# jstmn/cppflow

Hardware: AMD Instinct MI355X
Metric: LM-IK iterations/sec (seeds x waypoints) (higher is better)
Workload: dtype f32

## Files before the change

cppflow_amd/csrc/kernels_fused.h:

```cpp
#pragma once


__device__ __forceinline__ void load_target(const float* __restrict__ target, int w, float (&Rt)[9], float (&tt)[3]) {
    const float* t = target + (size_t)w * 7;
    tt[0] = t[0], tt[1] = t[1], tt[2] = t[2];
    quat_to_mat(t[3], t[4], t[5], t[6], Rt);
}

struct RowSummary {
    float pos_err = 0.f, rot_err = 0.f, cost = 0.f;
    int self_hit = 0, env_hit = 0, jl = 0;
};

template <int CTRL>
__device__ __forceinline__ float dpp_or_zero(float x) {
    return __builtin_bit_cast(float, __builtin_amdgcn_update_dpp(0, __builtin_bit_cast(int, x), CTRL, 0xf, 0xf, false));
}

template <bool IS_MAX>
__device__ __forceinline__ float wave_reduce_to_lane63(float v) {
    auto op = [](float a, float b) { return IS_MAX ? fmaxf(a, b) : a + b; };
    const float s1 = dpp_or_zero<0x111>(v), s2 = dpp_or_zero<0x112>(v), s3 = dpp_or_zero<0x113>(v);
    v = op(op(v, s1), op(s2, s3));
    v = op(v, dpp_or_zero<0x114>(v));
    v = op(v, dpp_or_zero<0x118>(v));
    v = op(v, dpp_or_zero<0x142>(v));
    v = op(v, dpp_or_zero<0x143>(v));
    return v;
}

__device__ __forceinline__ void lds_barrier() { asm volatile("s_waitcnt lgkmcnt(0)\n\ts_barrier" ::: "memory"); }

template <class RB>
__device__ __forceinline__ void block_seed_summary(const RB& rb, int W, size_t row, bool active, const float (&q)[RB::D],
                                                   const RowSummary& rs, float* __restrict__ out) {
    constexpr int D = RB::D;
    __shared__ float s_q[kBlock / 64][D];
    __shared__ float s_red[kBlock / 64][8];
    const int tid = threadIdx.x, lane = tid & 63, wave = tid >> 6;
    const float rad2deg = 57.29577951308232087680f;
    const int wps = W >> 6;
    if (wps > 1) {
        if (lane == 0) {
#pragma unroll
            for (int j = 0; j < D; ++j) s_q[wave][j] = q[j];
        }
        lds_barrier();
    }
    const bool seed_ends_here = ((wave + 1) & (wps - 1)) == 0;
    const bool has_next = active && !(lane == 63 && seed_ends_here);
    const int nw = wave + 1 < kBlock / 64 ? wave + 1 : wave;
    float mrev = 0.f, mpri = 0.f;
    float dq[D], wr[D];
#pragma unroll
    for (int j = 0; j < D; ++j) {
        float qn = dpp_or_zero<0x130>(q[j]);
        qn = (lane == 63) ? s_q[nw][j] : qn;
        dq[j] = wr[j] = qn - q[j];
    }
    wrap_pi_all<D>(wr);
#pragma unroll
    for (int j = 0; j < D; ++j) {
        const bool pr = rb.pris(j);
        const float a = nan_to_inf(pr ? fabsf(100.f * dq[j]) : fabsf(rad2deg * wr[j]));
        mpri = fmaxf(mpri, pr ? a : 0.f);
        mrev = fmaxf(mrev, pr ? 0.f : a);
    }
    float v[8] = {nan_to_inf(100.f * rs.pos_err), nan_to_inf(rad2deg * rs.rot_err), has_next ? mrev : 0.f, has_next ? mpri : 0.f,
                  (float)rs.self_hit, (float)rs.env_hit, (float)rs.jl, rs.cost};
#pragma unroll
    for (int k = 0; k < 8; ++k) v[k] = active ? v[k] : 0.f;
#pragma unroll
    for (int k = 0; k < 4; ++k) v[k] = wave_reduce_to_lane63<true>(v[k]);
#pragma unroll
    for (int k = 4; k < 8; ++k) v[k] = wave_reduce_to_lane63<false>(v[k]);
    float* o = out + ((uint32_t)row >> (31 - __builtin_clz((uint32_t)W))) * 8;
    if (wps == 1) {
        if (active && lane == 63) {
#pragma unroll
            for (int k = 0; k < 8; ++k) o[k] = v[k];
        }
        return;
    }
    if (lane == 63) {
#pragma unroll
        for (int k = 0; k < 8; ++k) s_red[wave][k] = v[k];
    }
    lds_barrier();
    if (active && lane == 63 && seed_ends_here) {
        for (int i = 1; i < wps; ++i) {
#pragma unroll
            for (int k = 0; k < 4; ++k) v[k] = fmaxf(v[k], s_red[wave - i][k]);
#pragma unroll
            for (int k = 4; k < 8; ++k) v[k] += s_red[wave - i][k];
        }
#pragma unroll
        for (int k = 0; k < 8; ++k) o[k] = v[k];
    }
}

#ifndef CPPF_LM_PACE
#define CPPF_LM_PACE 1
#endif
__device__ __forceinline__ void lm_pace(uint32_t t0, int k, int pace) {
    if (CPPF_LM_PACE == 0 || pace == 0) return;
    const int lag = (int)((uint32_t)__builtin_amdgcn_s_memrealtime() - t0) - k * pace, half = pace >> 1;
    if (lag > half)
        __builtin_amdgcn_s_setprio(3);
    else if (lag > 0)
        __builtin_amdgcn_s_setprio(2);
    else if (lag > -half)
        __builtin_amdgcn_s_setprio(1);
    else
        __builtin_amdgcn_s_setprio(0);
}

template <class RB>
__device__ __forceinline__ void lm_row_load(int W, const float* __restrict__ x_in, const float* __restrict__ target,
                                            size_t row, float (&q)[RB::D], float (&Rt)[9], float (&tt)[3]) {
    load_x<RB::D>(x_in, row, q);
    load_target(target, (int)((uint32_t)row % (uint32_t)W), Rt, tt);
}

#ifndef CPPF_LEAD_SINCOS
#define CPPF_LEAD_SINCOS 2
#endif
#ifndef CPPF_FIRST_LEAN
#define CPPF_FIRST_LEAN 1
#endif
template <class RB, bool LEAD, bool FIRST = false>
constexpr int lead_sincos() {
    return LEAD ? (FIRST && CPPF_LEAD_SINCOS == 2 ? 3 : CPPF_LEAD_SINCOS) : 0;
}
template <class RB, bool LEAD, bool FIRST = false>
__device__ __forceinline__ bool lm_row_iterate(const RB& rb, const LmK& prm, const cppf_lm_outputs& out, size_t row, bool last,
                                               const float (&Rt)[9], const float (&tt)[3], float* __restrict__ gate_lds,
                                               float (&q)[RB::D]) {
    constexpr int D = RB::D;
    float delta[D];
    bool conv = false;
    {
        float R[9], p[3], ax[D][3], og[D][3], J[6][D], e[6];
        fk_ee_axes<RB, lead_sincos<RB, LEAD, FIRST>()>(rb, q, R, p, ax, og);
        pose_error<LEAD>(Rt, tt, R, p, e);
        if constexpr (!LEAD) {
            if (prm.tol_pos2 > 0.f) {
                conv = dot3(e[3], e[4], e[5], e[3], e[4], e[5]) < prm.tol_pos2 && dot3(e[0], e[1], e[2], e[0], e[1], e[2]) < prm.tol_rot2;
                if (__builtin_amdgcn_ballot_w64(!conv) == 0ull) return true;
            }
        }
        jacobian_from_axes<RB>(rb, p, ax, og, J);
        float est = 0.f;
        if constexpr (D < 6) {
            lm_primal_solve<D>(J, e, prm.lm_lambda, prm.a_pos, prm.a_rot, delta);
        } else {
            float y[6];
            if constexpr (LEAD && CPPF_LEAN_BLOCK_SOLVE != 0)
                lm_dual_solve_y_blk<D>(J, e, prm.lam_r, prm.lam_p, y, est);
            else
                lm_dual_solve_y<D>(J, e, prm.lam_r, prm.lam_p, y, est);
            lm_dual_apply<D>(J, y, delta);
        }
        if constexpr (!LEAD) {
            if (last) {
                if (out.J_out) {
                    float* Jo = out.J_out + row * 6 * D;
#pragma unroll
                    for (int i = 0; i < 6; ++i)
#pragma unroll
                        for (int j = 0; j < D; ++j) Jo[i * D + j] = J[i][j] * (i < 3 ? prm.a_rot : prm.a_pos);
                }
                if (out.e_out) {
#pragma unroll
                    for (int i = 0; i < 6; ++i) out.e_out[row * 6 + i] = e[i] * (i < 3 ? prm.a_rot : prm.a_pos);
                }
            }
        }
        if constexpr (D >= 6) {
            bool flag = !conv && est > prm.gate_thr;
            if (__builtin_expect(__builtin_amdgcn_ballot_w64(flag) != 0ull, 0)) {
                if (prm.clamp && prm.gate_thr > -INFINITY) {
                    bool cut = false;
#pragma unroll
                    for (int j = 0; j < D; ++j) {
                        const float v = q[j] + delta[j];
                        cut |= (v < rb.lo(j)) | (v > rb.hi(j));
                    }
                    flag = flag && !cut;
                }
                if constexpr (LEAD) {
                    if (prm.gate_thr > -INFINITY) {
                        const float es2 = CPPF_FMA(prm.a_pos * prm.a_pos, dot3(e[3], e[4], e[5], e[3], e[4], e[5]),
                                                   prm.a_rot * prm.a_rot * dot3(e[0], e[1], e[2], e[0], e[1], e[2]));
                        flag = flag && est * est > prm.gate_rel2 * es2;
                    }
                }
                unsigned long long todo = __builtin_amdgcn_ballot_w64(flag);
                if (todo != 0ull) {
                    int rank = lm_gate_hand_over<D>(J, e, todo, gate_lds, flag);
                    lm_gate_solve<D>(prm.lam_r_d, prm.lam_p_d, todo, rank, gate_lds, flag, delta);
                    while ((todo = __builtin_amdgcn_ballot_w64(flag)) != 0ull) {
                        float R2[9], p2[3], ax2[D][3], og2[D][3], J2[6][D], e2[6];
#pragma unroll
                        for (int j = 0; j < D; ++j) asm volatile("" : "+v"(q[j]));
                        fk_ee_axes<RB, lead_sincos<RB, LEAD, FIRST>()>(rb, q, R2, p2, ax2, og2);
                        pose_error<LEAD>(Rt, tt, R2, p2, e2);
                        jacobian_from_axes<RB>(rb, p2, ax2, og2, J2);
                        rank = lm_gate_hand_over<D>(J2, e2, todo, gate_lds, flag);
                        lm_gate_solve<D>(prm.lam_r_d, prm.lam_p_d, todo, rank, gate_lds, flag, delta);
                    }
                }
            }
        }
    }
    if constexpr (!LEAD) {
        if (prm.tol_pos2 > 0.f) {
            if (!conv) {
#pragma unroll
                for (int j = 0; j < D; ++j) q[j] += delta[j];
                if (prm.clamp) clamp_row<RB>(rb, q);
            }
            return conv;
        }
    }
#pragma unroll
    for (int j = 0; j < D; ++j) q[j] += delta[j];
    if (prm.clamp) clamp_row<RB>(rb, q);
    return false;
}

template <class RB, int COLL>
__device__ __forceinline__ void lm_row_finish(const RB& rb, const CollK& co, const cppf_lm_outputs& out, float* lds, int tid,
                                              size_t row, const float (&Rt)[9], const float (&tt)[3], const float (&q)[RB::D],
                                              RowSummary& rs) {
    constexpr int D = RB::D;
    if (out.x_out) store_x<D>(out.x_out, row, q);
    const bool want_metrics = out.pos_err_m || out.rot_err_rad || out.seed_summary;
    if constexpr (COLL != 0) {
        const bool do_self = out.self_mask || out.min_self || out.ext_cost || out.seed_summary;
        const bool do_env = out.env_mask || out.min_env || out.ext_cost || out.seed_summary;
        rs.jl = jlim_hit<D>(co, q);
        CollOut c;
        auto metrics = [&](float (&R)[9], float (&p)[3]) {
            if (want_metrics) {
                fk_fixed_ee(rb, R, p);
                pose_metrics(Rt, tt, R, p, rs.pos_err, rs.rot_err);
                if (out.pos_err_m) out.pos_err_m[row] = rs.pos_err;
                if (out.rot_err_rad) out.rot_err_rad[row] = rs.rot_err;
            }
        };
        if constexpr (RB::kStatic) {
            constexpr int L = RB::Table::L > 0 ? RB::Table::L : 1;
            float wc[L][3], wh[L][3];
            {
                float R[9], p[3];
                capsule_fk_static<RB>(rb, q, R, p, wc, wh);
                metrics(R, p);
            }
            c = collide_tests_static<RB, COLL == 2>(co, wc, wh, do_self, do_env);
        } else {
            {
                float R[9], p[3];
                fk_capsules_to_lds<RB>(rb, co, q, lds, tid, R, p);
                metrics(R, p);
            }
            c = collide_from_lds<COLL == 2>(co, lds, tid, do_self, do_env);
        }
        rs.self_hit = c.self_hit, rs.env_hit = c.env_hit;
        rs.cost = 100.f * (float)rs.jl + 1000.f * (float)c.env_hit + 1000.f * (float)c.self_hit;
        write_coll_outputs(row, c, rs.jl, out.self_mask, out.env_mask, out.jlim_mask, out.ext_cost, out.min_self,
                           out.min_env);
    } else {
        if (want_metrics) {
            float R[9], p[3];
            fk_ee<RB>(rb, q, R, p);
            pose_metrics(Rt, tt, R, p, rs.pos_err, rs.rot_err);
            if (out.pos_err_m) out.pos_err_m[row] = rs.pos_err;
            if (out.rot_err_rad) out.rot_err_rad[row] = rs.rot_err;
        }
    }
}

template <class RB>
constexpr int lm_waves() {
    return RB::kStatic ? (RB::D <= 7 ? 4 : 3) : (RB::D <= 6 ? 4 : (RB::D <= 8 ? 3 : 2));
}

template <class T>
__device__ __forceinline__ T* as_global(T* p) {
    return (T*)(__attribute__((address_space(1))) T*)p;
}

typedef const __attribute__((address_space(4))) BatchItemK* BatchItemPtr;

__device__ __forceinline__ BatchItemPtr fused_item(const void* table, uint32_t& blk) {
    typedef const __attribute__((address_space(4))) char* CPtr;
    blk = blockIdx.x;
    BatchItemPtr itp = (BatchItemPtr)((CPtr)__builtin_amdgcn_kernarg_segment_ptr() + __builtin_offsetof(FusedArgs, single));
    if (table) {
        const CPtr tab = (CPtr)(uintptr_t)table;
        const __attribute__((address_space(4))) BatchHeadK* hd = (const __attribute__((address_space(4))) BatchHeadK*)tab;
        uint32_t b = 0, begin = 0;
#pragma unroll
        for (int i = 0; i < CPPF_MAX_BATCH - 1; ++i) {
            const uint32_t e = hd->block_end[i];
            const bool past = blk >= e;
            b = past ? (uint32_t)(i + 1) : b;
            begin = past ? e : begin;
        }
        blk -= begin;
        itp = (BatchItemPtr)(tab + sizeof(BatchHeadK)) + b;
    }
    return itp;
}

__device__ __forceinline__ cppf_lm_outputs fused_outputs(BatchItemPtr itp) {
    cppf_lm_outputs o;
    o.x_out = as_global(itp->out.x_out), o.J_out = as_global(itp->out.J_out), o.e_out = as_global(itp->out.e_out);
    o.pos_err_m = as_global(itp->out.pos_err_m), o.rot_err_rad = as_global(itp->out.rot_err_rad);
    o.self_mask = as_global(itp->out.self_mask), o.env_mask = as_global(itp->out.env_mask), o.jlim_mask = as_global(itp->out.jlim_mask);
    o.ext_cost = as_global(itp->out.ext_cost), o.min_self = as_global(itp->out.min_self), o.min_env = as_global(itp->out.min_env);
    o.seed_summary = as_global(itp->out.seed_summary), o.n_iters = as_global(itp->out.n_iters);
    return o;
}

template <class RB, int COLL>
__global__ __launch_bounds__(kBlock) __attribute__((amdgpu_waves_per_eu(lm_waves<RB>(), lm_waves<RB>()))) void lm_fused_kernel(const ChainK ch, const CollK co, const LmK prm,
                                                          const BatchItemK single, const void* table) {
    extern __shared__ float lds[];
    (void)single;
    constexpr int D = RB::D;
    __shared__ float s_gate[kBlock / 64][GateLds<D>::kFloats];
    static_assert(sizeof(s_gate) + (kBlock / 64) * (D + 8) * sizeof(float) <= fused_static_lds_bound(D), "fused_static_lds_bound is stale");
    const RB rb{ch, co};
    uint32_t blk;
    const BatchItemPtr itp = fused_item(table, blk);
    const cppf_lm_outputs out = fused_outputs(itp);
    const int tid = threadIdx.x;
    const size_t row = (size_t)(blk * (unsigned)kBlock + (unsigned)tid);
    const bool active = row < (size_t)itp->n;
    float q[D];
#pragma unroll
    for (int j = 0; j < D; ++j) q[j] = 0.f;
    RowSummary rs;
    if (active) {
        float Rt[9], tt[3];
        lm_row_load<RB>(itp->W, as_global(itp->x_in), as_global(itp->target), row, q, Rt, tt);
        float chk = tt[0] + tt[1] + tt[2];
#pragma unroll
        for (int j = 0; j < D; ++j) chk += q[j];
#pragma unroll
        for (int k = 0; k < 9; ++k) chk += Rt[k];
        unsigned long long bad_mask = __builtin_amdgcn_ballot_w64(!(fabsf(chk) < INFINITY));
        asm volatile("" : "+s"(bad_mask));
        float* const gate_lds = s_gate[__builtin_amdgcn_readfirstlane(tid >> 6)];
        const uint32_t pace_t0 = (CPPF_LM_PACE != 0 && prm.pace_ticks != 0) ? (uint32_t)__builtin_amdgcn_s_memrealtime() : 0u;
        int iters = 0, it = 0;
        if (!(prm.tol_pos2 > 0.f)) {
            if (prm.n_steps >= 2) {
                (void)lm_row_iterate<RB, CPPF_FIRST_LEAN != 0, true>(rb, prm, out, row, false, Rt, tt, gate_lds, q);
                it = 1;
            }
            for (; it < prm.n_steps - 1; ++it) {
                lm_pace(pace_t0, it, prm.pace_ticks);
                (void)lm_row_iterate<RB, true>(rb, prm, out, row, false, Rt, tt, gate_lds, q);
            }
            iters = it;
            lm_pace(pace_t0, it, prm.pace_ticks);
        }
        for (; it < prm.n_steps; ++it) {
            const bool conv = lm_row_iterate<RB, false>(rb, prm, out, row, it == prm.n_steps - 1, Rt, tt, gate_lds, q);
            iters += conv ? 0 : 1;
            if (prm.tol_pos2 > 0.f && __builtin_amdgcn_ballot_w64(!conv) == 0ull) break;
        }
        int tid_b = threadIdx.x;
        asm volatile("" : "+v"(tid_b));
        const size_t row_b = (size_t)(blk * (unsigned)kBlock + (unsigned)tid_b);
        if (out.n_iters) out.n_iters[row_b] = iters;
        if ((bad_mask >> (tid_b & 63)) & 1ull) {
#pragma unroll
            for (int j = 0; j < D; ++j) q[j] = __builtin_nanf("");
        }
        lm_pace(pace_t0, prm.n_steps, prm.pace_ticks);
        lm_row_finish<RB, COLL>(rb, co, out, lds, tid_b, row_b, Rt, tt, q, rs);
    }
    if constexpr (COLL != 0) {
        if (out.seed_summary) {
            int tid_c = threadIdx.x;
            asm volatile("" : "+v"(tid_c));
            block_seed_summary<RB>(rb, itp->W, (size_t)(blk * (unsigned)kBlock + (unsigned)tid_c), active, q, rs, out.seed_summary);
        }
    }
}

template <class RB, bool WANT_MIN>
__global__ __launch_bounds__(kBlock, CPPF_WAVES_COLL) void collision_kernel(const ChainK ch, const CollK co, int n,
                                                           const float* __restrict__ x, uint8_t* self_mask,
                                                           uint8_t* env_mask, uint8_t* jlim_mask, float* ext_cost,
                                                           float* min_self, float* min_env, const StepGateK gate, int gate_W) {
    extern __shared__ float lds[];
    constexpr int D = RB::D;
    const RB rb{ch, co};
    const int tid = threadIdx.x;
    const size_t row = (size_t)blockIdx.x * kBlock + tid;
    if (row >= (size_t)n) return;
    if (gate.ctl != nullptr && !step_open(gate, (int)(row / (size_t)gate_W))) return;
    float q[D], R[9], p[3];
    load_x<D>(x, row, q);
    const bool do_self = self_mask || min_self || ext_cost;
    const bool do_env = env_mask || min_env || ext_cost;
    CollOut c;
    c.min_self = c.min_env = INFINITY;
    c.self_hit = c.env_hit = 0;
    if (do_self || do_env) c = collide_row<RB, WANT_MIN>(rb, co, q, lds, tid, R, p, do_self, do_env);
    write_coll_outputs(row, c, jlim_hit<D>(co, q), self_mask, env_mask, jlim_mask, ext_cost, min_self, min_env);
}

template <int D, bool ENV>
__global__ __launch_bounds__(kBlock) void distances_kernel(const ChainK ch, const CollK co, int n,
                                                           const float* __restrict__ x, float blo0, float blo1,
                                                           float blo2, float bhi0, float bhi1, float bhi2,
                                                           float* __restrict__ dists) {
    extern __shared__ float lds[];
    using RB = DynRobot<D>;
    const RB rb{ch, co};
    const int tid = threadIdx.x;
    const size_t row = (size_t)blockIdx.x * kBlock + tid;
    if (row >= (size_t)n) return;
    float q[D], R[9], p[3];
    load_x<D>(x, row, q);
    fk_capsules_to_lds<RB>(rb, co, q, lds, tid, R, p);
    if constexpr (ENV) {
        const float lo[3] = {blo0, blo1, blo2}, hi[3] = {bhi0, bhi1, bhi2};
        for (int c = 0; c < co.ncaps; ++c) {
            float wc[3], wh[3];
            lds_capsule(lds, tid, c, wc, wh);
            dists[row * co.ncaps + c] = seg_box_dist(wc, wh, lo, hi) - co.cap_r[c];
        }
    } else {
        for (int pi = 0; pi < co.npairs; ++pi) {
            const int a = co.pair_a[pi], b = co.pair_b[pi];
            float ca[3], ha[3], cb[3], hb[3];
            lds_capsule(lds, tid, a, ca, ha);
            lds_capsule(lds, tid, b, cb, hb);
            dists[row * co.npairs + pi] =
                seg_seg_dist(ca, ha, cb, hb, co.cap_a[a], co.cap_ia[a], co.cap_a[b], co.cap_ia[b]) - (co.cap_r[a] + co.cap_r[b]);
        }
    }
}

template <int D>
__global__ __launch_bounds__(kBlock) void fk_kernel(const ChainK ch, const CollK co, int n, const float* __restrict__ x,
                                                    float* __restrict__ poses) {
    using RB = DynRobot<D>;
    const RB rb{ch, co};
    const size_t row = (size_t)blockIdx.x * kBlock + threadIdx.x;
    if (row >= (size_t)n) return;
    float q[D], R[9], p[3], qt[4];
    load_x<D>(x, row, q);
    fk_ee<RB>(rb, q, R, p);
    mat_to_quat(R, qt);
    float* o = poses + row * 7;
    o[0] = p[0], o[1] = p[1], o[2] = p[2], o[3] = qt[0], o[4] = qt[1], o[5] = qt[2], o[6] = qt[3];
}

template <int D>
__global__ __launch_bounds__(kBlock) void jacobian_kernel(const ChainK ch, const CollK co, int n,
                                                          const float* __restrict__ x, float* __restrict__ Jout) {
    using RB = DynRobot<D>;
    const RB rb{ch, co};
    const size_t row = (size_t)blockIdx.x * kBlock + threadIdx.x;
    if (row >= (size_t)n) return;
    float q[D], R[9], p[3], ax[D][3], og[D][3], J[6][D];
    load_x<D>(x, row, q);
    fk_ee_axes<RB>(rb, q, R, p, ax, og);
    jacobian_from_axes<RB>(rb, p, ax, og, J);
    float* Jo = Jout + row * 6 * D;
#pragma unroll
    for (int i = 0; i < 6; ++i)
#pragma unroll
        for (int j = 0; j < D; ++j) Jo[i * D + j] = J[i][j];
}

template <int D>
__global__ __launch_bounds__(kBlock) void pose_errors_kernel(const ChainK ch, const CollK co, int n, int W,
                                                             const float* __restrict__ x,
                                                             const float* __restrict__ target, float* __restrict__ e_out,
                                                             float* __restrict__ cur_out) {
    using RB = DynRobot<D>;
    const RB rb{ch, co};
    const size_t row = (size_t)blockIdx.x * kBlock + threadIdx.x;
    if (row >= (size_t)n) return;
    float q[D], R[9], p[3], Rt[9], tt[3], e[6];
    load_x<D>(x, row, q);
    load_target(target, (int)(row % (size_t)W), Rt, tt);
    fk_ee<RB>(rb, q, R, p);
    pose_error(Rt, tt, R, p, e);
    if (e_out) {
#pragma unroll
        for (int i = 0; i < 6; ++i) e_out[row * 6 + i] = e[i];
    }
    if (cur_out) {
        float qt[4];
        mat_to_quat(R, qt);
        float* o = cur_out + row * 7;
        o[0] = p[0], o[1] = p[1], o[2] = p[2], o[3] = qt[0], o[4] = qt[1], o[5] = qt[2], o[6] = qt[3];
    }
}

template <int D>
__global__ __launch_bounds__(kBlock) void pose_metrics_kernel(const ChainK ch, const CollK co, int n, int W,
                                                              const float* __restrict__ x,
                                                              const float* __restrict__ target,
                                                              float* __restrict__ pos_err, float* __restrict__ rot_err) {
    using RB = DynRobot<D>;
    const RB rb{ch, co};
    const size_t row = (size_t)blockIdx.x * kBlock + threadIdx.x;
    if (row >= (size_t)n) return;
    float q[D], R[9], p[3], Rt[9], tt[3], pe, re;
    load_x<D>(x, row, q);
    load_target(target, (int)(row % (size_t)W), Rt, tt);
    fk_ee<RB>(rb, q, R, p);
    pose_metrics(Rt, tt, R, p, pe, re);
    if (pos_err) pos_err[row] = pe;
    if (rot_err) rot_err[row] = re;
}

__device__ __forceinline__ float clamp_joint(const ChainK& ch, int j, float v) {
    return v != v ? v : fminf(fmaxf(v, ch.lo[j]), ch.hi[j]);
}

__global__ __launch_bounds__(kBlock) void clamp_kernel(const ChainK ch, size_t total, float* __restrict__ x) {
    const size_t i = (size_t)blockIdx.x * kBlock + threadIdx.x;
    if (i >= total) return;
    const int j = (int)(i % (size_t)ch.ndof);
    x[i] = clamp_joint(ch, j, x[i]);
}

template <int D>
__global__ __launch_bounds__(64) void seed_validity_kernel(const ChainK ch, const CollK co, int S, int W,
                                                           const float* __restrict__ x,
                                                           const float* __restrict__ target, float* __restrict__ out) {
    using RB = DynRobot<D>;
    const RB rb{ch, co};
    const int s = blockIdx.x;
    if (s >= S) return;
    const float rad2deg = 57.29577951308232087680f;
    float mp = 0.f, mr = 0.f, mrev = 0.f, mpri = 0.f;
    for (int w = threadIdx.x; w < W; w += 64) {
        const size_t row = (size_t)s * W + w;
        float q[D], R[9], p[3], Rt[9], tt[3], pe, re;
        load_x<D>(x, row, q);
        load_target(target, w, Rt, tt);
        fk_ee<RB>(rb, q, R, p);
        pose_metrics(Rt, tt, R, p, pe, re);
        mp = fmaxf(mp, nan_to_inf(100.f * pe));
        mr = fmaxf(mr, nan_to_inf(rad2deg * re));
        if (w + 1 < W) {
            float qn[D], dq[D], wr[D];
            load_x<D>(x, row + 1, qn);
#pragma unroll
            for (int j = 0; j < D; ++j) dq[j] = wr[j] = qn[j] - q[j];
            wrap_pi_all<D>(wr);
#pragma unroll
            for (int j = 0; j < D; ++j) {
                if (rb.pris(j))
                    mpri = fmaxf(mpri, nan_to_inf(fabsf(100.f * dq[j])));
                else
                    mrev = fmaxf(mrev, nan_to_inf(fabsf(rad2deg * wr[j])));
            }
        }
    }
#pragma unroll
    for (int off = 32; off > 0; off >>= 1) {
        mp = fmaxf(mp, __shfl_xor(mp, off, 64));
        mr = fmaxf(mr, __shfl_xor(mr, off, 64));
        mrev = fmaxf(mrev, __shfl_xor(mrev, off, 64));
        mpri = fmaxf(mpri, __shfl_xor(mpri, off, 64));
    }
    if (threadIdx.x == 0) {
        out[s * 4 + 0] = mp, out[s * 4 + 1] = mr, out[s * 4 + 2] = mrev, out[s * 4 + 3] = mpri;
    }
}
```

Before: 79.13 billion.

## Reduce seed summary with integer bit-pattern maxima and packed hit counts

```diff
diff --git a/cppflow_amd/csrc/kernels_fused.h b/cppflow_amd/csrc/kernels_fused.h
--- a/cppflow_amd/csrc/kernels_fused.h
+++ b/cppflow_amd/csrc/kernels_fused.h
@@ -8,20 +8,20 @@
 }
 
 struct RowSummary {
-    float pos_err = 0.f, rot_err = 0.f, cost = 0.f;
+    float pos_err = 0.f, rot_err = 0.f;
     int self_hit = 0, env_hit = 0, jl = 0;
 };
 
 template <int CTRL>
-__device__ __forceinline__ float dpp_or_zero(float x) {
-    return __builtin_bit_cast(float, __builtin_amdgcn_update_dpp(0, __builtin_bit_cast(int, x), CTRL, 0xf, 0xf, false));
+__device__ __forceinline__ uint32_t dpp_or_zero(uint32_t x) {
+    return (uint32_t)__builtin_amdgcn_update_dpp(0, (int)x, CTRL, 0xf, 0xf, true);
 }
 
 template <bool IS_MAX>
-__device__ __forceinline__ float wave_reduce_to_lane63(float v) {
-    auto op = [](float a, float b) { return IS_MAX ? fmaxf(a, b) : a + b; };
-    const float s1 = dpp_or_zero<0x111>(v), s2 = dpp_or_zero<0x112>(v), s3 = dpp_or_zero<0x113>(v);
-    v = op(op(v, s1), op(s2, s3));
+__device__ __forceinline__ uint32_t wave_reduce_to_lane63(uint32_t v) {
+    auto op = [](uint32_t a, uint32_t b) { return IS_MAX ? __builtin_elementwise_max(a, b) : a + b; };
+    v = op(v, dpp_or_zero<0x111>(v));
+    v = op(v, dpp_or_zero<0x112>(v));
     v = op(v, dpp_or_zero<0x114>(v));
     v = op(v, dpp_or_zero<0x118>(v));
     v = op(v, dpp_or_zero<0x142>(v));
@@ -29,16 +29,45 @@
     return v;
 }
 
+__device__ __forceinline__ uint32_t nonneg_bits_nan_to_inf(float x) {
+    return __builtin_elementwise_min(__builtin_bit_cast(uint32_t, x), 0x7f800000u);
+}
+
 __device__ __forceinline__ void lds_barrier() { asm volatile("s_waitcnt lgkmcnt(0)\n\ts_barrier" ::: "memory"); }
+
+template <class RB>
+__device__ __forceinline__ void joint_change_maxima(const RB& rb, const float (&dq)[RB::D], const float (&wr)[RB::D], uint32_t& mrev,
+                                                    uint32_t& mpri) {
+    const float rad2deg = 57.29577951308232087680f;
+    mrev = mpri = 0u;
+#pragma unroll
+    for (int j = 0; j < RB::D; ++j) {
+        if (rb.pris(j))
+            mpri = __builtin_elementwise_max(mpri, __builtin_bit_cast(uint32_t, 100.f * fabsf(dq[j])));
+        else
+            mrev = __builtin_elementwise_max(mrev, __builtin_bit_cast(uint32_t, rad2deg * fabsf(wr[j])));
+    }
+    mrev = __builtin_elementwise_min(mrev, 0x7f800000u), mpri = __builtin_elementwise_min(mpri, 0x7f800000u);
+}
+
+template <class RB, bool = RB::kStatic>
+struct MayHavePrismatic {
+    static constexpr bool value = true;
+};
+template <class RB>
+struct MayHavePrismatic<RB, true> {
+    static constexpr bool value = RB::Table::pris_mask != 0;
+};
 
 template <class RB>
 __device__ __forceinline__ void block_seed_summary(const RB& rb, int W, size_t row, bool active, const float (&q)[RB::D],
                                                    const RowSummary& rs, float* __restrict__ out) {
     constexpr int D = RB::D;
+    static_assert(kBlock <= 256, "a seed's hit counts (<= W <= kBlock) are packed into 10-bit fields");
     __shared__ float s_q[kBlock / 64][D];
-    __shared__ float s_red[kBlock / 64][8];
-    const int tid = threadIdx.x, lane = tid & 63, wave = tid >> 6;
-    const float rad2deg = 57.29577951308232087680f;
+    __shared__ uint32_t s_red[kBlock / 64][5];
+    const int tid = threadIdx.x, lane = tid & 63, wave = __builtin_amdgcn_readfirstlane(tid >> 6);
+    const float rad2deg = 57.29577951308232087680f, pi = 3.14159265358979323846f;
     const int wps = W >> 6;
     if (wps > 1) {
         if (lane == 0) {
@@ -50,52 +79,51 @@
     const bool seed_ends_here = ((wave + 1) & (wps - 1)) == 0;
     const bool has_next = active && !(lane == 63 && seed_ends_here);
     const int nw = wave + 1 < kBlock / 64 ? wave + 1 : wave;
-    float mrev = 0.f, mpri = 0.f;
     float dq[D], wr[D];
 #pragma unroll
     for (int j = 0; j < D; ++j) {
-        float qn = dpp_or_zero<0x130>(q[j]);
-        qn = (lane == 63) ? s_q[nw][j] : qn;
-        dq[j] = wr[j] = qn - q[j];
-    }
-    wrap_pi_all<D>(wr);
-#pragma unroll
-    for (int j = 0; j < D; ++j) {
-        const bool pr = rb.pris(j);
-        const float a = nan_to_inf(pr ? fabsf(100.f * dq[j]) : fabsf(rad2deg * wr[j]));
-        mpri = fmaxf(mpri, pr ? a : 0.f);
-        mrev = fmaxf(mrev, pr ? 0.f : a);
-    }
-    float v[8] = {nan_to_inf(100.f * rs.pos_err), nan_to_inf(rad2deg * rs.rot_err), has_next ? mrev : 0.f, has_next ? mpri : 0.f,
-                  (float)rs.self_hit, (float)rs.env_hit, (float)rs.jl, rs.cost};
-#pragma unroll
-    for (int k = 0; k < 8; ++k) v[k] = active ? v[k] : 0.f;
-#pragma unroll
-    for (int k = 0; k < 4; ++k) v[k] = wave_reduce_to_lane63<true>(v[k]);
-#pragma unroll
-    for (int k = 4; k < 8; ++k) v[k] = wave_reduce_to_lane63<false>(v[k]);
+        const float qn = __builtin_bit_cast(float, __builtin_amdgcn_update_dpp(__builtin_bit_cast(int, s_q[nw][j]), __builtin_bit_cast(int, q[j]),
+                                                                               0x130, 0xf, 0xf, false));
+        dq[j] = qn - q[j];
+        wr[j] = (dq[j] + pi) - pi;
+    }
+    uint32_t mrev, mpri;
+    joint_change_maxima<RB>(rb, dq, wr, mrev, mpri);
+    mrev = has_next ? mrev : 0u, mpri = has_next ? mpri : 0u;
+    if (__builtin_expect(__builtin_amdgcn_ballot_w64(mrev >= __builtin_bit_cast(uint32_t, 171.f)) != 0ull, 0)) {
+#pragma unroll
+        for (int j = 0; j < D; ++j) wr[j] = dq[j];
+        wrap_pi_all<D>(wr);
+        uint32_t mr, mp;
+        joint_change_maxima<RB>(rb, dq, wr, mr, mp);
+        mrev = has_next ? mr : 0u;
+    }
+    uint32_t v[5] = {nonneg_bits_nan_to_inf(100.f * fabsf(rs.pos_err)), nonneg_bits_nan_to_inf(rad2deg * fabsf(rs.rot_err)), mrev, mpri,
+                     (uint32_t)rs.jl | (uint32_t)rs.env_hit << 10 | (uint32_t)rs.self_hit << 20};
+#pragma unroll
+    for (int k = 0; k < 3; ++k) v[k] = wave_reduce_to_lane63<true>(v[k]);
+    if constexpr (MayHavePrismatic<RB>::value) v[3] = wave_reduce_to_lane63<true>(v[3]);
+    v[4] = wave_reduce_to_lane63<false>(v[4]);
     float* o = out + ((uint32_t)row >> (31 - __builtin_clz((uint32_t)W))) * 8;
-    if (wps == 1) {
-        if (active && lane == 63) {
-#pragma unroll
-            for (int k = 0; k < 8; ++k) o[k] = v[k];
-        }
-        return;
-    }
-    if (lane == 63) {
-#pragma unroll
-        for (int k = 0; k < 8; ++k) s_red[wave][k] = v[k];
-    }
-    lds_barrier();
+    if (wps > 1) {
+        if (lane == 63) {
+#pragma unroll
+            for (int k = 0; k < 5; ++k) s_red[wave][k] = v[k];
+        }
+        lds_barrier();
+    }
     if (active && lane == 63 && seed_ends_here) {
+#pragma unroll 1
         for (int i = 1; i < wps; ++i) {
 #pragma unroll
-            for (int k = 0; k < 4; ++k) v[k] = fmaxf(v[k], s_red[wave - i][k]);
-#pragma unroll
-            for (int k = 4; k < 8; ++k) v[k] += s_red[wave - i][k];
-        }
-#pragma unroll
-        for (int k = 0; k < 8; ++k) o[k] = v[k];
+            for (int k = 0; k < 4; ++k) v[k] = __builtin_elementwise_max(v[k], s_red[wave - i][k]);
+            v[4] += s_red[wave - i][4];
+        }
+#pragma unroll
+        for (int k = 0; k < 4; ++k) o[k] = __builtin_bit_cast(float, v[k]);
+        const float jl = (float)(v[4] & 1023u), env = (float)((v[4] >> 10) & 1023u), self = (float)(v[4] >> 20);
+        o[4] = self, o[5] = env, o[6] = jl;
+        o[7] = 100.f * jl + 1000.f * env + 1000.f * self;
     }
 }
 
@@ -267,7 +295,6 @@
             c = collide_from_lds<COLL == 2>(co, lds, tid, do_self, do_env);
         }
         rs.self_hit = c.self_hit, rs.env_hit = c.env_hit;
-        rs.cost = 100.f * (float)rs.jl + 1000.f * (float)c.env_hit + 1000.f * (float)c.self_hit;
         write_coll_outputs(row, c, rs.jl, out.self_mask, out.env_mask, out.jlim_mask, out.ext_cost, out.min_self,
                            out.min_env);
     } else {
```

New measurement: 80.58 billion, median of 6. +1.8%, better.
